# TimoLassmann/tagdust

Hardware: AMD Instinct MI355X
Metric: reads/s (150 bp, 8-barcode arch) (higher is better)
Workload: dtype f32

## Files before the change

### tagdust_amd/csrc/td_jit.h

```cpp
#pragma once
#include <string>
#include <vector>
#include "../../include/tagdust_hip.h"
#include "td_device.h"

struct TdSpecKnobs {
	int block = 512;
	int min_waves = 4;
	int lsum_oob = 1;
	int rt_min = 16;
	int groupcols = 18;
	int groupcols_fwd = 12;
	int prune = 1;
	int prune_sfx = 1;
	int restart = -1;
	int firstseg = -1;
	int trie_sh = 2;
	int profile = 0;
	int prune_stats = -1;
	std::string extra_opts;
};
TdSpecKnobs td_spec_knobs(void);

#define TD_PRUNE_TABLES 16
#define TD_PRUNE_RESTART_MAX 4

struct TdSpecPlan {
	TdSpecKnobs k;
	int S = 0, H = 0, C = 0;
	std::vector<int> col_off, hmm_off;
	std::vector<int> group, group_f;
	std::vector<int> pure_last, drop_m;
	std::vector<int> bw_off;
	int64_t halves = 0;
	std::vector<int> rt, rt_b;
	std::vector<int> base;
	std::vector<float> hi, lo, nv;
	bool trie_on = false;
	int trie_sh = 1, trie_n_share = 0;
	std::vector<int> trie_ord;
	int first_n = 0;
	int prune_segs = 0;
	int sfx_first = 0;
	float prune_z = 0.0f;
	int restart = 0;
};
TdSpecPlan td_spec_plan(const td_model_desc* m, const TdSpecKnobs& k);

float td_spec_prune_z(const td_model_desc* m, int n_seg, int sfx_first);
void td_spec_prune_tables(const td_model_desc* m, const TdSpecPlan& p, int lcap, int stride, std::vector<float>& tab);
void td_spec_layout(TdSpecLayout& L, const TdSpecPlan& p, int lmax);
int td_spec_compile(const td_model_desc* m, const TdSpecPlan& p, int lsum_oob, int window, std::vector<char>& code, std::string& log,
                    uint64_t* key_out = nullptr, bool key_only = false);
int td_spec_compiles_started(void);
```

### tagdust_amd/csrc/td_jit.hip

```cpp
#include <hip/hip_runtime.h>
#include <hip/hiprtc.h>
#include <math.h>
#include <stdio.h>
#include <string.h>
#include <stdlib.h>

#include <atomic>
#include <map>
#include <mutex>
#include <string>
#include <vector>

#include "../../include/tagdust_hip.h"
#include "td_device.h"
#include <unistd.h>
#include <sys/stat.h>
#include <sys/types.h>
#include "td_embedded_src.h"
#include "td_jit.h"

static std::string flit(float v)
{
	if (isinf(v)) return v < 0 ? "(-__builtin_inff())" : "__builtin_inff()";
	if (v != v) return "__builtin_nanf(\"\")";
	char buf[64];
	snprintf(buf, sizeof buf, "%af", (double)v);
	return buf;
}

TdSpecKnobs td_spec_knobs(void)
{
	TdSpecKnobs k;
	auto num = [](const char* name, int unset) { const char* e = getenv(name); return e ? atoi(e) : unset; };
	auto flag = [](const char* name, int unset) -> int { const char* e = getenv(name); return e ? atoi(e) != 0 : unset; };
	if (const int v = num("TD_SPEC_BLOCK", 0); v >= 64 && v <= 1024 && v % 64 == 0) k.block = v;
	if (const int v = num("TD_SPEC_MINWAVES", 0); v >= 1 && v <= 8) k.min_waves = v;
	if (const int v = num("TD_SPEC_GROUPCOLS", 0); v > 0) k.groupcols = v;
	k.groupcols_fwd = num("TD_SPEC_GROUPCOLS_FWD", k.groupcols_fwd);
	k.rt_min = num("TD_SPEC_RT_MIN", k.rt_min);
	k.trie_sh = num("TD_SPEC_TRIE_SH", k.trie_sh);
	k.profile = num("TD_SPEC_PROFILE", k.profile);
	k.lsum_oob = flag("TD_SPEC_LSUM_OOB", k.lsum_oob);
	k.prune = flag("TD_SPEC_PRUNE", k.prune);
	k.prune_sfx = flag("TD_SPEC_PRUNE_SFX", k.prune_sfx);
	k.restart = flag("TD_SPEC_RESTART", k.restart);
	k.firstseg = flag("TD_SPEC_FIRSTSEG", k.firstseg);
	k.prune_stats = flag("TD_SPEC_PRUNE_STATS", k.prune_stats);
	if (const char* e = getenv("TD_SPEC_EXTRA_OPTS")) k.extra_opts = e;
	return k;
}

namespace {
int pure_last(const td_model_desc* m, int j, int col_off)
{
	for (int f = 0; f < m->n_hmm[j]; f++) {
		const int q = col_off + f * m->n_col[j] + m->n_col[j] - 1;
		if (!(m->trans[q * 9 + 4] == -INFINITY) || !(m->trans[q * 9 + 3] == -INFINITY)) return 0;
	}
	return 1;
}

int rt_prefix(const td_model_desc* m, int j, int col_off, int* base , float* hi, float* lo, float* nv, int min_hmms)
{
	const int n = m->n_hmm[j], nc = m->n_col[j];
	if (n < min_hmms) return 0;
	auto match_type = [&](int q, int* b, float* h, float* l, float* v) -> bool {
		const float* e = m->eM + (size_t)q * 5;
		for (int x = 0; x < 4; x++) {
			const float other = e[(x + 1) & 3];
			bool ok = !(e[x] == other);
			for (int y = 0; y < 4 && ok; y++) if (y != x && !(e[y] == other)) ok = false;
			if (ok) { *b = x; *h = e[x]; *l = other; *v = e[4]; return true; }
		}
		return false;
	};
	int b0; float h0, l0, v0;
	if (!match_type(col_off, &b0, &h0, &l0, &v0)) return 0;
	int f = 0;
	for (; f < n; f++) {
		bool ok = true;
		for (int g = 0; g < nc && ok; g++) {
			const int q = col_off + f * nc + g, q0 = col_off + g;
			if (memcmp(m->trans + (size_t)q * 9, m->trans + (size_t)q0 * 9, 36) || memcmp(m->eI + (size_t)q * 5, m->eI + (size_t)q0 * 5, 20) ||
			    memcmp(&m->sM[q], &m->sM[q0], 4) || memcmp(&m->sI[q], &m->sI[q0], 4)) { ok = false; break; }
			int b; float h, l, v;
			if (!match_type(q, &b, &h, &l, &v) || memcmp(&h, &h0, 4) || memcmp(&l, &l0, 4) || memcmp(&v, &v0, 4)) { ok = false; break; }
			base[q] = b;
		}
		if (!ok) break;
	}
	*hi = h0; *lo = l0; *nv = v0;
	return f >= min_hmms ? f : 0;
}

int group_size(int n_hmm, int n_col, int target)
{
	int maxf = target / n_col;
	if (maxf < 1) maxf = 1;
	if (maxf > n_hmm) maxf = n_hmm;
	const int groups = (n_hmm + maxf - 1) / maxf;
	return (n_hmm + groups - 1) / groups;
}

int first_labels(const td_model_desc* m, int firstseg)
{
	const int H = m->H, n0 = m->n_hmm[0];
	const int mode = firstseg >= 0 ? firstseg : H > 32;
	if (!mode) return 0;
	if (n0 < 2 || n0 >= H) return 0;
	for (int v = 0; v < n0; v++)
		for (int u = 0; u < v; u++) if (m->A[u * H + v] == 1.0f) return 0;
	for (int w = n0; w < H; w++) {
		int c = 0;
		for (int u = 0; u < n0; u++) c += m->A[u * H + w] == 1.0f;
		if (c != 0 && c != n0) return 0;
	}
	return n0;
}

bool read_like(const td_model_desc* m, int j, int co)
{
	if (m->n_hmm[j] != 1 || m->n_col[j] != 1) return false;
	const float* t = m->trans + (size_t)co * 9;
	for (int k = 0; k < 9; k++) if (k != TD_II && k != TD_ISKIP && t[k] > -INFINITY) return false;
	return m->sM[co] == -INFINITY && m->sI[co] > -INFINITY && t[TD_II] > -INFINITY && t[TD_ISKIP] > -INFINITY;
}
}

TdSpecPlan td_spec_plan(const td_model_desc* m, const TdSpecKnobs& k)
{
	TdSpecPlan p;
	const int S = m->S, H = m->H, C = m->C;
	p.k = k; p.S = S; p.H = H; p.C = C;
	p.col_off.resize(S); p.hmm_off.resize(S);
	for (int j = 0, co = 0, ho = 0; j < S; co += m->n_hmm[j] * m->n_col[j], ho += m->n_hmm[j], j++) { p.col_off[j] = co; p.hmm_off[j] = ho; }
	p.group.resize(S); p.group_f.resize(S); p.pure_last.resize(S); p.drop_m.resize(S); p.bw_off.resize(H);
	for (int j = 0; j < S; j++) {
		p.group[j] = group_size(m->n_hmm[j], m->n_col[j], k.groupcols);
		p.group_f[j] = group_size(m->n_hmm[j], m->n_col[j], k.groupcols_fwd > 0 ? k.groupcols_fwd : k.groupcols);
		p.pure_last[j] = pure_last(m, j, p.col_off[j]);
	}
	int cols = 0;
	for (int j = 0; j < S; j++) {
		p.drop_m[j] = m->n_col[j] >= 2 && p.pure_last[j];
		for (int f = 0; f < m->n_hmm[j]; f++) { p.bw_off[p.hmm_off[j] + f] = cols; cols += 2 * (m->n_col[j] - p.pure_last[j]) - p.drop_m[j]; }
	}
	p.halves = cols;
	p.rt.assign(S, 0); p.rt_b.assign(S, 0); p.base.assign(C, 0);
	p.hi.assign(S, 0.0f); p.lo.assign(S, 0.0f); p.nv.assign(S, 0.0f);
	for (int j = 0; j < S; j++) {
		const int pre = rt_prefix(m, j, p.col_off[j], p.base.data(), &p.hi[j], &p.lo[j], &p.nv[j], k.rt_min);
		if (pre > 0) {
			p.group_f[j] = p.group[j];
			p.rt[j] = pre / p.group[j] * p.group[j];
			p.rt_b[j] = p.rt[j];
		} else {
			p.rt_b[j] = rt_prefix(m, j, p.col_off[j], p.base.data(), &p.hi[j], &p.lo[j], &p.nv[j], 2);
		}
	}
	{
		const int sh = k.trie_sh;
		bool on = p.rt[0] > 0 && sh >= 1 && m->n_col[0] >= sh + 2;
		std::vector<int> ord;
		int n_share = 0;
		if (on) {
			const int G = p.group[0], NC0 = m->n_col[0];
			std::map<std::vector<int>, std::vector<int>> cls;
			for (int f = 0; f < p.rt[0]; f++) {
				std::vector<int> key;
				for (int g = NC0 - sh; g < NC0; g++) key.push_back(p.base[(size_t)(p.col_off[0] + f * NC0 + g)]);
				cls[key].push_back(f);
			}
			std::vector<int> left;
			for (auto& kv : cls) {
				const std::vector<int>& v = kv.second;
				const size_t full = v.size() / (size_t)G * (size_t)G;
				for (size_t i = 0; i < full; i++) ord.push_back(v[i]);
				for (size_t i = full; i < v.size(); i++) left.push_back(v[i]);
			}
			n_share = (int)ord.size() / G;
			for (int f : left) ord.push_back(f);
			if (n_share == 0) on = false;
		}
		if (!on) { ord.assign(1, 0); n_share = 0; }
		p.trie_on = on; p.trie_sh = on ? sh : 1; p.trie_n_share = n_share; p.trie_ord = ord;
	}
	p.first_n = first_labels(m, k.firstseg);
	p.prune_segs = 0; p.sfx_first = S;
	if (k.prune && H - p.first_n <= 32) {
		int first = -1, last = -1;
		for (int j = 0; j < S; j++) if (read_like(m, j, p.col_off[j])) { if (first < 0) first = j; last = j; }
		if (first > 0) p.prune_segs = first;
		bool single = k.prune_sfx && last >= 0 && last < S - 1;
		for (int j = last + 1; single && j < S; j++) if (m->n_hmm[j] != 1) single = false;
		if (single) p.sfx_first = last + 1;
	}
	p.prune_z = td_spec_prune_z(m, p.prune_segs, p.sfx_first);
	if (p.prune_segs <= 0 || p.prune_segs > TD_PRUNE_RESTART_MAX || (p.sfx_first < S && S - p.sfx_first > TD_PRUNE_RESTART_MAX)) p.restart = 0;
	else if (k.restart >= 0) p.restart = k.restart;
	else p.restart = p.col_off[p.prune_segs] >= 48;
	return p;
}

static std::string td_spec_model_section(const td_model_desc* m, const TdSpecPlan& p, int lsum_oob, int window)
{
	std::string s;
	char buf[256];
	const int S = m->S, H = m->H, C = m->C;
	int req = 0;
	for (int j = 0; j < S; j++) if (m->seg_type[j] == 'F') req += m->finger_len[j];
	snprintf(buf, sizeof buf, "#define TDS_BLOCK %d\n#define TDS_MIN_WAVES %d\n", p.k.block, p.k.min_waves);
	s += buf;
	snprintf(buf, sizeof buf, "#define TDS_LSUM_OOB %d\n", lsum_oob != 0);
	s += buf;
	snprintf(buf, sizeof buf, "#define TDS_WINDOW %d\n", window != 0);
	s += buf;
	snprintf(buf, sizeof buf, "#define TDS_PROFILE %d\n", p.k.profile);
	s += buf;
	snprintf(buf, sizeof buf, "#define TD_S %d\n#define TD_H %d\n#define TD_C %d\n#define TD_REQ_FINGER %d\n", S, H, C, req);
	s += buf;
	s += "struct GCol { float t[9]; float sM, sI; float eM[5]; float eI[5]; };\n";
	auto int_array = [&](const char* name, const std::vector<int>& v) {
		s += std::string("static constexpr int ") + name + "[" + std::to_string(v.size()) + "] = {";
		for (size_t i = 0; i < v.size(); i++) { s += std::to_string(v[i]); if (i + 1 < v.size()) s += ","; }
		s += "};\n";
	};
	int_array("kNHmm", std::vector<int>(m->n_hmm, m->n_hmm + S)); int_array("kNCol", std::vector<int>(m->n_col, m->n_col + S));
	int_array("kColOff", p.col_off); int_array("kHmmOff", p.hmm_off);
	int_array("kRtB", p.rt_b);
	s += std::string("static constexpr bool kTrieOn = ") + (p.trie_on ? "true" : "false") + ";\n";
	s += "static constexpr int kTrieSH = " + std::to_string(p.trie_sh) + ";\n";
	s += "static constexpr int kTrieNShare = " + std::to_string(p.trie_n_share) + ";\n";
	int_array("kTrieOrd", p.trie_ord);
	int_array("kGroup", p.group); int_array("kGroupF", p.group_f); int_array("kPureLast", p.pure_last); int_array("kDropM", p.drop_m); int_array("kBwOff", p.bw_off);
	int_array("kRt", p.rt); int_array("kBase", p.base);
	auto float_array = [&](const char* name, const std::vector<float>& v) {
		s += std::string("static constexpr float ") + name + "[" + std::to_string(v.size()) + "] = {";
		for (size_t i = 0; i < v.size(); i++) { s += flit(v[i]); if (i + 1 < v.size()) s += ","; }
		s += "};\n";
	};
	float_array("kHi", p.hi); float_array("kLo", p.lo); float_array("kNv", p.nv);
	s += "static constexpr float kSkip[" + std::to_string(S) + "] = {";
	for (int j = 0; j < S; j++) { s += flit(m->skip[j]); if (j + 1 < S) s += ","; }
	s += "};\n";
	s += "static constexpr float kBg[5] = {";
	for (int i = 0; i < 5; i++) { s += flit(m->bg[i]); if (i < 4) s += ","; }
	s += "};\n";
	const float stay_arg = (float)(1.0 - (1.0 / (double)(float)m->avg_len));
	const float exit_arg = (float)(1.0 / (double)(float)m->avg_len);
	s += "static constexpr float kRStay = " + flit(stay_arg == 0.0f ? -INFINITY : (float)log((double)stay_arg)) + ";\n";
	s += "static constexpr float kRExit = " + flit(exit_arg == 0.0f ? -INFINITY : (float)log((double)exit_arg)) + ";\n";
	s += "static constexpr GCol kCols[" + std::to_string(C) + "] = {\n";
	for (int k = 0; k < C; k++) {
		s += " {{";
		for (int t = 0; t < 9; t++) { s += flit(m->trans[k * 9 + t]); if (t < 8) s += ","; }
		s += "}," + flit(m->sM[k]) + "," + flit(m->sI[k]) + ",{";
		for (int e = 0; e < 5; e++) { s += flit(m->eM[k * 5 + e]); if (e < 4) s += ","; }
		s += "},{";
		for (int e = 0; e < 5; e++) { s += flit(m->eI[k * 5 + e]); if (e < 4) s += ","; }
		s += "}},\n";
	}
	s += "};\n";
	s += "static constexpr unsigned kHinfo[" + std::to_string(H) + "] = {";
	for (int h = 0; h < H; h++) {
		const int seg = m->label[h] & 0xFFFF, f = (m->label[h] >> 16) & 0x7FFF;
		unsigned v = (unsigned)(unsigned char)m->seg_type[seg] | ((unsigned)seg << 8) | ((unsigned)f << 16);
		if (m->seg_type[seg] == 'B' && f == m->n_hmm[seg] - 1) v |= 0x80000000u;
		snprintf(buf, sizeof buf, "0x%08xu%s", v, h + 1 < H ? "," : "");
		s += buf;
	}
	s += "};\n";
	std::vector<int> poff(H + 1, 0), pidx;
	for (int v = 0; v < H; v++) {
		poff[v] = (int)pidx.size();
		for (int u = 0; u < v; u++) if (m->A[u * H + v] == 1.0f) pidx.push_back(u);
	}
	poff[H] = (int)pidx.size();
	if (pidx.empty()) pidx.push_back(0);
	int_array("kPredOff", poff); int_array("kPredIdx", pidx);
	const int first_n = p.first_n;
	std::vector<int> pfirst(H, 0), poff2(H + 1, 0), pidx2;
	for (int v = 0; v < H; v++) {
		poff2[v] = (int)pidx2.size();
		for (int i = poff[v]; i < poff[v + 1]; i++) {
			if (pidx[i] < first_n) pfirst[v] = 1; else pidx2.push_back(pidx[i]);
		}
	}
	poff2[H] = (int)pidx2.size();
	if (pidx2.empty()) pidx2.push_back(0);
	s += "static constexpr int kFirstN = " + std::to_string(first_n) + ";\n";
	int_array("kPredFirst", pfirst); int_array("kPredOff2", poff2); int_array("kPredIdx2", pidx2);
	std::vector<int> runs;
	for (int v = first_n; v < H; v++) {
		bool same = v > first_n && pfirst[v] == pfirst[v - 1] && poff2[v + 1] - poff2[v] == poff2[v] - poff2[v - 1];
		for (int k = 0; same && k < poff2[v + 1] - poff2[v]; k++) same = pidx2[poff2[v] + k] == pidx2[poff2[v - 1] + k];
		if (!same) runs.push_back(v - first_n);
	}
	runs.push_back(H - first_n);
	s += "static constexpr int kPruneSegs = " + std::to_string(p.prune_segs) + ";\n";
	s += "static constexpr int kSfxFirst = " + std::to_string(p.sfx_first) + ";\n";
	s += "static constexpr float kPruneZ = " + flit(p.prune_z) + ";\n";
	if (p.k.prune_stats >= 0) s += std::string("#define TDS_PRUNE_STATS ") + (p.k.prune_stats ? "1" : "0") + "\n";
	s += std::string("#ifndef TDS_RESTART\n#define TDS_RESTART ") + (p.restart ? "1" : "0") + "\n#endif\n";
	s += "static constexpr int kNRuns = " + std::to_string((int)runs.size() - 1) + ";\n";
	int_array("kRunOff", runs);
	return s;
}

static std::string td_spec_full_source(const td_model_desc* m, const TdSpecPlan& p, int lsum_oob, int window)
{
	std::string src = "#ifndef __HIPCC_RTC__\n#include <hip/hip_runtime.h>\n#endif\n#include <stdint.h>\n";
	src += kSrcDeviceH;
	src += "\n";
	src += kSrcArtifact;
	src += "\n";
	src += td_spec_model_section(m, p, lsum_oob, window);
	src += kSrcSpecKernel;
	return src;
// ... 193 lines not shown
```

### tagdust_amd/csrc/td_spec_kernel.inc

```

#ifndef TDS_BLOCK
#define TDS_BLOCK 512
#endif
#ifndef TDS_MIN_WAVES
#define TDS_MIN_WAVES 4
#endif
#define TDS_REG_H 32
#define TDS_WPB (TDS_BLOCK / TD_WAVE)
#define NEG_INF (-__builtin_inff())
#define DEV __device__ __forceinline__

#define MODE_GET_LABEL 1
#define MODE_ARCH_COMP 5
#define OUT_SUCCESS 0
#define OUT_ARCH_MISMATCH 1
#define OUT_TOO_SHORT 2
#define OUT_BAR_FINGER_NOT_FOUND 3
#define OUT_MATCHES_ARTIFACTS 5
#define OUT_LOW_COMPLEXITY 6
#define N_OUTCOME_SLOTS 8
#define TDS_DIAG(k) (N_OUTCOME_SLOTS + 256 + ((k) - 192))

#ifndef TDS_LSUM_OOB
#define TDS_LSUM_OOB 1
// ... 109 lines not shown
	const int c1 = (e0 == e1) + (e2 == e1) + (e3 == e1);
	const int c2 = (e0 == e2) + (e1 == e2) + (e3 == e2);
	const int c3 = (e0 == e3) + (e1 == e3) + (e2 == e3);
	float lo = e0;
	int best = c0;
	if (c1 > best) { lo = e1; best = c1; }
	if (c2 > best) { lo = e2; best = c2; }
	if (c3 > best) { lo = e3; best = c3; }
	float r = lo;
	if (e0 != lo) r = k.m0 ? e0 : r;
	if (e1 != lo) r = k.m1 ? e1 : r;
	if (e2 != lo) r = k.m2 ? e2 : r;
	if (e3 != lo) r = k.m3 ? e3 : r;
	if (e4 != lo) r = k.m4 ? e4 : r;
	return r;
}
#define EMIT_M(col, k) emit(kCols[col].eM[0], kCols[col].eM[1], kCols[col].eM[2], kCols[col].eM[3], kCols[col].eM[4], k)
#define EMIT_I(col, k) emit(kCols[col].eI[0], kCols[col].eI[1], kCols[col].eI[2], kCols[col].eI[3], kCols[col].eI[4], k)
DEV float emit_rt(const int b, const float hi, const float lo, const float nv, const BaseMask& k, const int x)
{
	const float r = (x == b) ? hi : lo;
	return k.m4 ? nv : r;
}

#ifndef TDS_PROFILE
#define TDS_PROFILE 0
#endif
#define TDS_PHASE(k) do { if (TDS_PROFILE) { const long long t_ = (long long)__builtin_readcyclecounter(); \
	if (lane == 0) atomicAdd(&ka.counters[TDS_DIAG(240 + (k))], (unsigned long long)(t_ - tprof)); tprof = t_; } } while (0)

#ifndef TDS_WINDOW
#define TDS_WINDOW 0
#endif
constexpr bool kMaskDP = TD_H - kFirstN <= TDS_REG_H;

struct Wv {
	uint32_t* pmask;
	int nwm;
	uint8_t* slot;
	int lane, len, lmax, tmax, tmin;
	float* bm;
	uint8_t* ba;
	int cut;
	int cutS;
	const float* wa;
	const float* wb;
	int sstop;
	int sstopS;
	const float* wc;
	const float* wd;
	mutable int bad;
	bool rb_on, rf_on;
	float* rs;
	float* hb;
	int rWf;
	int rW;
	const float* bwt;
	const float* fbs;
	unsigned long long* stats;
	long long* tprof;
	const float* ptab;
	int pstride;
	const float* qr;
	const float* pr;
};

#ifndef TDS_LATE_CS
#define TDS_LATE_CS 1
#endif
#ifndef TDS_PF_DIST
#define TDS_PF_DIST 4
#endif
#ifndef TDS_PF_COLS
#define TDS_PF_COLS 2
#endif
#ifndef TDS_LDP
#define TDS_LDP 2
#endif
#ifndef TDS_LDT
#define TDS_LDT 4
#endif
#ifndef TDS_SCAN_B
#define TDS_SCAN_B 8
#endif
#ifndef TDS_PRUNE_TT
#define TDS_PRUNE_TT (-88.0f)
#endif
#ifndef TDS_PRUNE_MARGIN
#define TDS_PRUNE_MARGIN 1
#endif
#ifndef TDS_PRUNE_BGAP
#define TDS_PRUNE_BGAP 5.0f
#endif
#ifndef TDS_PRUNE_STATS
#define TDS_PRUNE_STATS 0
#endif

constexpr int cmin(int a, int b) { return a < b ? a : b; }
constexpr int pf_dist(int cols, bool rt) { return (!rt && cols <= TDS_PF_COLS) ? TDS_PF_DIST : 1; }
template <int D> struct IC { static constexpr int v = D; };
constexpr bool label_leading(int h)
{
	for (int j = 0; j < kPruneSegs; j++) if (h >= kHmmOff[j] && h < kHmmOff[j] + kNHmm[j]) return true;
	return false;
}
template <int PD, int D, typename F>
DEV void ring_block(F& step, const int base)
{
	if constexpr (D < PD) { step(IC<D>{}, base + D); ring_block<PD, D + 1>(step, base); }
}
template <int PD, int D, typename F>
DEV void ring_rest(F& step, const int base, const int iend)
{
	if constexpr (D < PD - 1) { if (base + D <= iend) { step(IC<D>{}, base + D); ring_rest<PD, D + 1>(step, base, iend); } }
}

template <int J, bool RT>
DEV void bwd_row(const int fa, const float (&Mn)[kNCol[J]], const float (&In)[kNCol[J]], const float Pn,
                 const BaseMask& kc, const int c, const BaseMask& kx, const int xi, SV (&Mc)[kNCol[J]], SV (&Ic)[kNCol[J]])
{
#define EM(gcol, mask, xval) (RT ? emit_rt(kBase[colr + (gcol)], kHi[J], kLo[J], kNv[J], mask, xval) : EMIT_M(col0 + (gcol), mask))
	constexpr int NC = kNCol[J];
	constexpr int K = NC - 1;
	const int col0 = kColOff[J] + (RT ? 0 : fa) * NC;
	const int colr = kColOff[J] + fa * NC;
	(void)colr;
	SV Dp = sv_none();
	{
		const int q = col0 + K;
		const SV M = addc(sv(Pn), kCols[q].t[7]);
		SV I = addc(sv(Pn), kCols[q].t[8]);
		I = lsum(I, addv(addc(sv(Mn[K]), kCols[q].t[4]), EM(K, kc, c)));
		I = lsum(I, addv(addc(sv(In[K]), kCols[q].t[3]), EMIT_I(q, kc)));
		Mc[K] = M; Ic[K] = I;
	}
#pragma unroll
	for (int g = K - 1; g >= 0; --g) {
		const int q = col0 + g;
		const float epc = EM(g + 1, kc, c);
		const float eic = EMIT_I(q, kc);
		SV M = addc(addv(sv(Mn[g + 1]), epc), kCols[q].t[0]);
		SV I = addv(addc(sv(In[g]), kCols[q].t[3]), eic);
		lsum2(M, addc(sv(Pn), kCols[q].t[7]), I, addc(sv(Pn), kCols[q].t[8]));
		lsum2(M, addc(addv(sv(In[g]), eic), kCols[q].t[1]), I, addv(addc(sv(Mn[g + 1]), kCols[q].t[4]), epc));
		SV D = addc(Dp, kCols[q].t[5]);
		lsum2(M, addc(Dp, kCols[q].t[2]), D, addc(addv(Mc[g + 1], EM(g + 1, kx, xi)), kCols[q].t[6]));
		Mc[g] = M; Ic[g] = I; Dp = D;
	}
#undef EM
}

template <int J, bool RT, int GT, int GB>
DEV void bwd_cols(const int fa, const float (&Mn)[kNCol[J]], const float (&In)[kNCol[J]], const float Pn,
                  const BaseMask& kc, const int c, const BaseMask& kx, const int xi, SV (&Mc)[kNCol[J]], SV (&Ic)[kNCol[J]], SV& Dp)
{
#define EM(gcol, mask, xval) (RT ? emit_rt(kBase[colr + (gcol)], kHi[J], kLo[J], kNv[J], mask, xval) : EMIT_M(col0 + (gcol), mask))
	constexpr int NC = kNCol[J];
	constexpr int K = NC - 1;
	const int col0 = kColOff[J] + (RT ? 0 : fa) * NC;
	const int colr = kColOff[J] + fa * NC;
	(void)colr;
	if constexpr (GT == K) {
		const int q = col0 + K;
		const SV M = addc(sv(Pn), kCols[q].t[7]);
		SV I = addc(sv(Pn), kCols[q].t[8]);
		I = lsum(I, addv(addc(sv(Mn[K]), kCols[q].t[4]), EM(K, kc, c)));
// ... 559 lines not shown
			ub_term(mi, ni, addc(Io, kCols[q].t[3]));
			ub_term(mi, ni, addc(Mo, kCols[q].t[1]));
			ub_term(md, nd, addc(Mcu, kCols[qp].t[2]));
			ub_term(md, nd, addc(Du, kCols[qp].t[5]));
			Mc[g] = nm ? si(NEG_INF, ub_done(mm, nm) + em) : si_none();
			Ic[g] = ni ? si(NEG_INF, ub_done(mi, ni) + ei) : si_none();
			Dc = nd ? si(NEG_INF, ub_done(md, nd)) : si_none();
		}
	}
#pragma unroll
	for (int g = 0; g < NC; g++) {
		Mlo[g] = Mc[g].z ? NEG_INF : Mc[g].lo; Mhi[g] = Mc[g].z ? NEG_INF : Mc[g].hi;
		Ilo[g] = Ic[g].z ? NEG_INF : Ic[g].lo; Ihi[g] = Ic[g].z ? NEG_INF : Ic[g].hi;
	}
}

template <int J, int GC>
DEV void fstair_dispatch(const int gc, float (&Mlo)[kNCol[J]], float (&Mhi)[kNCol[J]], float (&Ilo)[kNCol[J]], float (&Ihi)[kNCol[J]], const float Pm, const BaseMask& kc)
{
	if constexpr (kNCol[J] > TDS_STAIR_STATIC_COLS) {
		fstair_step<J, -2>(gc, Mlo, Mhi, Ilo, Ihi, Pm, kc);
	} else if constexpr (GC <= kNCol[J]) {
		if (gc == GC) fstair_step<J, GC>(gc, Mlo, Mhi, Ilo, Ihi, Pm, kc);
		else fstair_dispatch<J, GC + 1>(gc, Mlo, Mhi, Ilo, Ihi, Pm, kc);
	}
}

template <int J>
DEV void fwd_stair(const Wv& w, const uint8_t* __restrict__ codes, const float* __restrict__ P, const int q_lo, const int q_hi)
{
	constexpr int NC = kNCol[J];
	float hi0 = NEG_INF;
	{
		const float* gf = w.ptab + (int64_t)(12 + J - kSfxFirst) * w.pstride;
		const int t = q_lo - 1;
		for (int k0 = 1; k0 <= t; k0 += 8) {
			float pr[8];
#pragma unroll
			for (int u = 0; u < 8; u++) { const int k = k0 + u; pr[u] = w.pr[((k <= t) ? t - k : 0) * TD_WAVE + w.lane]; }
			__builtin_amdgcn_sched_barrier(0);
#pragma unroll
			for (int u = 0; u < 8; u++) { const int k = k0 + u; if (k <= t) hi0 = fmaxf(hi0, uload(gf, k) + pr[u]); }
		}
		hi0 = fminf(hi0 + (__logf((float)(t > 1 ? t : 1)) + 0.02f), w.fbs[t]);
	}
	float Mlo[NC], Mhi[NC], Ilo[NC], Ihi[NC];
#pragma unroll
	for (int g = 0; g < NC; g++) { Mlo[g] = NEG_INF; Ilo[g] = NEG_INF; Mhi[g] = hi0; Ihi[g] = hi0; }
	int gc = 0;
	int closed_at = -1;
	auto close_check = [&](const int steps_done) __attribute__((always_inline)) {
		if (gc < NC) {
			bool cl = true;
#pragma unroll
			for (int g = 0; g < NC; g++) if (g == gc) cl = same(si(Mlo[g], Mhi[g])) && same(si(Ilo[g], Ihi[g]));
			if (__builtin_amdgcn_ballot_w64(!cl) == 0) { gc++; if (gc == NC) closed_at = steps_done; }
		}
	};
	int c_n = codes[q_lo * TD_WAVE + w.lane];
	float Pm_n = P[(q_lo - 1) * TD_WAVE + w.lane];
	for (int i = q_lo; i < q_hi; ++i) {
		const int c = c_n;
		const float Pm = Pm_n;
		{
			const int ip = (i + 1 < q_hi) ? i + 1 : i;
			c_n = codes[ip * TD_WAVE + w.lane];
			Pm_n = P[(ip - 1) * TD_WAVE + w.lane];
		}
		close_check(i - q_lo); close_check(i - q_lo);
		fstair_dispatch<J, 0>(gc, Mlo, Mhi, Ilo, Ihi, Pm, mk_mask(c));
	}
	close_check(q_hi - q_lo); close_check(q_hi - q_lo);
	if (gc < NC) w.bad |= 32;
	if (TDS_PRUNE_STATS && w.lane == 0) {
		const int st = closed_at >= 0 ? closed_at : q_hi - q_lo;
		atomicAdd(&w.stats[TDS_DIAG(194)], (unsigned long long)st); atomicAdd(&w.stats[TDS_DIAG(195)], 1ull);
		atomicMax(&w.stats[TDS_DIAG(192)], (unsigned long long)st);
	}
	float* rs = w.rs + (int64_t)kColOff[J] * 2 * TD_WAVE + w.lane;
#pragma unroll
	for (int g = 0; g < NC; g++) { rs[(2 * g) * TD_WAVE] = Mlo[g]; rs[(2 * g + 1) * TD_WAVE] = Ilo[g]; }
}

template <int J, int NF, bool RT>
DEV void fwd_group(const Wv& w, const uint8_t* __restrict__ codes, const float* __restrict__ P,
                   float* __restrict__ Cs, const float* __restrict__ PB, const uint8_t* __restrict__ BW,
                   float* __restrict__ DP, float* __restrict__ TOTAL, const float b, const int f0)
{
	const bool first = (f0 == 0);
#define EM(gcol, mask, xval) (RT ? emit_rt(kBase[colr + (gcol)], kHi[J], kLo[J], kNv[J], mask, xval) : EMIT_M(col0 + (gcol), mask))
	constexpr int NC = kNCol[J];
	constexpr int K = NC - 1;
	constexpr bool pure = kPureLast[J] != 0;
	constexpr int NS = NC - kPureLast[J];
	constexpr int DM = kDropM[J];
	constexpr int NSF = NS - DM;
	constexpr int ROWH = 2 * NS - DM;
	constexpr int NQ = NSF / 2;
	constexpr int NT = NSF & 1;
	constexpr bool skip_live = LIVE(kSkip[J]);
	float Mp[NF][NC], Ip[NF][NC], tot[NF];
#pragma unroll
	for (int f = 0; f < NF; f++) {
		tot[f] = NEG_INF;
#pragma unroll
		for (int g = 0; g < NC; g++) { Mp[f][g] = NEG_INF; Ip[f][g] = NEG_INF; }
	}
	if (TDS_RESTART && J >= kSfxFirst && w.rf_on) {
		const float* rs = w.rs + (int64_t)kColOff[J] * 2 * TD_WAVE + w.lane;
#pragma unroll
		for (int g = 0; g < NC; g++) { Mp[0][g] = rs[(2 * g) * TD_WAVE]; Ip[0][g] = rs[(2 * g + 1) * TD_WAVE]; }
	}
	constexpr bool p_init = (J == 0);
	const bool resumed = TDS_RESTART && (J >= kSfxFirst) && w.rf_on;
	const int i0 = resumed ? w.sstop - (TD_S - 1 - J) * (w.rWf + 1) : 1;
	float Pm = p_init ? 0.0f : P[(i0 - 1) * TD_WAVE + w.lane];
	constexpr int PD = pf_dist(NF * NC, RT);
	const int pmax = (w.tmax >= 1) ? w.tmax : 1;
	int c_q[PD];
	float Pi_q[PD], cs_q[PD], pb_q[PD], bm_q[PD], ik_q[PD][NF];
	int ba_q[PD];
	float MB_q[PD][NF][NSF + 1], IB_q[PD][NF][NSF + 1];
	constexpr bool pb_init = (J == TD_S - 1);
#define PBR(pos) (pb_init ? (((pos) == w.len + 1) ? 0.0f : NEG_INF) : PB[(pos) * TD_WAVE + w.lane])
#define BWROW(f_, pos_) (BW + ((int64_t)kBwOff[kHmmOff[J] + f0 + (f_)] * w.lmax + (int64_t)((pos_) - 1) * ROWH) * (TD_WAVE * 4))
#define TDS_FWD_FILL(d, p_raw) { \
		const int p_ = ((p_raw) <= pmax) ? (p_raw) : pmax; \
		c_q[d] = codes[p_ * TD_WAVE + w.lane]; \
		Pi_q[d] = p_init ? NEG_INF : P[p_ * TD_WAVE + w.lane]; \
		if (!first) cs_q[d] = Cs[p_ * TD_WAVE + w.lane]; \
		if (pure) pb_q[d] = PBR(p_ + 1); \
		if (own_sum && !first) { bm_q[d] = w.bm[p_ * TD_WAVE + w.lane]; ba_q[d] = w.ba[p_ * TD_WAVE + w.lane]; } \
		const bool rows_ = !((J >= kSfxFirst) && p_ < w.sstop);    \
_Pragma("unroll") \
		for (int f = 0; f < NF; f++) { \
			if (DM && rows_) ik_q[d][f] = ld1(BWROW(f, p_) + NSF * (TD_WAVE * 8), w.lane); \
			if (PD > 1 && rows_) { \
_Pragma("unroll") \
				for (int q = 0; q < NQ; q++) { \
					MB_q[d][f][2 * q] = ldk(BWROW(f, p_) + q * (TD_WAVE * 16), w.lane, 16, 0); IB_q[d][f][2 * q] = ldk(BWROW(f, p_) + q * (TD_WAVE * 16), w.lane, 16, 1); \
					MB_q[d][f][2 * q + 1] = ldk(BWROW(f, p_) + q * (TD_WAVE * 16), w.lane, 16, 2); IB_q[d][f][2 * q + 1] = ldk(BWROW(f, p_) + q * (TD_WAVE * 16), w.lane, 16, 3); \
				} \
				if (NT) { MB_q[d][f][NSF - 1] = ldk(BWROW(f, p_) + NQ * (TD_WAVE * 16), w.lane, 8, 0); IB_q[d][f][NSF - 1] = ldk(BWROW(f, p_) + NQ * (TD_WAVE * 16), w.lane, 8, 1); } \
			} \
		} \
	}
	constexpr bool own_sum = (J == 0) && (kFirstN > 0);
	float lacc[NF];
	uint32_t mbits[NF];
#pragma unroll
	for (int f = 0; f < NF; f++) { lacc[f] = 0.0f; mbits[f] = 0u; }
#pragma unroll
	for (int d = 0; d < PD; d++) {
		cs_q[d] = NEG_INF; pb_q[d] = 0.0f; bm_q[d] = -1.0f; ba_q[d] = 0;
#pragma unroll
		for (int f = 0; f < NF; f++) ik_q[d][f] = NEG_INF;
		TDS_FWD_FILL(d, i0 + d)
	}

	const int iend = (J < kPruneSegs && w.cut < w.tmax) ? w.cut : w.tmax;
	const int itail = (J == kPruneSegs && kPruneSegs > 0) ? w.cut + 1 : w.tmax + 1;
	(void)itail;
	if (i0 > 1 && kMaskDP && !own_sum) {
#pragma unroll
		for (int f = 0; f < NF; f++) {
			if (w.lane == 0) for (int wd = 0; wd < ((i0 - 1) >> 5); wd++) w.pmask[(kHmmOff[J] + f0 + f) * w.nwm + wd] = 0u;
			mbits[f] = 0u;
		}
	}
	auto step_cs = [&](auto dtag, auto cstag, const int i) __attribute__((always_inline)) {
		constexpr int d_ = decltype(dtag)::v;
		constexpr bool want_cs = decltype(cstag)::v != 0;
		const int c = c_q[d_];
		const float Pi = Pi_q[d_];
		const float pb = pb_q[d_];
		SV cs; cs.v = cs_q[d_]; cs.z = RT ? false : first;
		float bm = bm_q[d_];
		int ba = ba_q[d_];
		f32x4 cb[NF][NQ + 1];
		f32x2 ct[NF];
		const bool sfx_skip = (J >= kSfxFirst) && i < w.sstop;
		float ik[NF];
#pragma unroll
		for (int f = 0; f < NF; f++) {
			if constexpr (PD == 1) {
				const uint8_t* bw = BW + ((int64_t)kBwOff[kHmmOff[J] + f0 + f] * w.lmax + (int64_t)(i - 1) * ROWH) * (TD_WAVE * 4);
				if (!sfx_skip) {
#pragma unroll
					for (int p = 0; p < NQ; p++) cb[f][p] = ld4(bw + p * (TD_WAVE * 16), w.lane);
					if (NT) ct[f] = ld2(bw + NQ * (TD_WAVE * 16), w.lane);
				}
			} else {
#pragma unroll
				for (int p = 0; p < NQ; p++) cb[f][p] = f32x4{ MB_q[d_][f][2 * p], IB_q[d_][f][2 * p], MB_q[d_][f][2 * p + 1], IB_q[d_][f][2 * p + 1] };
				if (NT) ct[f] = f32x2{ MB_q[d_][f][NSF - 1], IB_q[d_][f][NSF - 1] };
			}
			ik[f] = ik_q[d_][f];
		}
		TDS_FWD_FILL(d_, i + PD)
		const int dn_ = (d_ + 1) % PD;
		const int c_n = c_q[dn_];
		const float pb_n = pb_q[dn_];
		float ik_n[NF];
#pragma unroll
		for (int f = 0; f < NF; f++) ik_n[f] = ik_q[dn_][f];
		float lpost[NF];
#pragma unroll
		for (int f = 0; f < NF; f++) lpost[f] = NEG_INF;
		const bool tail = (J == kPruneSegs && kPruneSegs > 0) && i >= itail;
		if (i <= w.len) {
			const SV PmS = sv(tail ? NEG_INF : Pm);
			const SV PiS = sv(tail ? NEG_INF : Pi);
			const BaseMask kc = mk_mask(c);
#pragma unroll
			for (int f = 0; f < NF; f++) {
				const int col0 = kColOff[J] + (RT ? 0 : (f0 + f)) * NC;
				const int colr = kColOff[J] + (f0 + f) * NC;
				(void)colr;
				const int h = kHmmOff[J] + f0 + f;
				SV Mc[NC], Ic[NC];
				SV Dc = sv_none();
				const float ei0 = EMIT_I(col0, kc);
				{
					const int q = col0;
					const SV M = addv(addc(PmS, kCols[q].sM), EM(0, kc, c));
					SV I = addc(PmS, kCols[q].sI);
					if (tail && LIVE(kCols[q].sI)) {
						if (!(Ip[f][0] + kCols[q].t[3] >= uload(w.wa, i))) w.bad |= 1;
					}
					I = lsum(I, addc(sv(Ip[f][0]), kCols[q].t[3]));
					I = lsum(I, addc(sv(Mp[f][0]), kCols[q].t[1]));
					I = addv(I, ei0);
					if (want_cs) { cs = lsum(cs, addc(M, kCols[q].t[7])); cs = lsum(cs, addc(I, kCols[q].t[8])); }
					Mc[0] = M; Ic[0] = I;
				}
#pragma unroll
				for (int g = 1; g <= K; ++g) {
					const int q = col0 + g, qp = q - 1;
					SV M = addc(PmS, kCols[q].sM);
					SV I = addc(PmS, kCols[q].sI);
					lsum2(M, addc(sv(Mp[f][g - 1]), kCols[qp].t[0]), I, addc(sv(Ip[f][g]), kCols[q].t[3]));
					lsum2(M, addc(sv(Ip[f][g - 1]), kCols[qp].t[4]), I, addc(sv(Mp[f][g]), kCols[q].t[1]));
					SV D = addc(Mc[g - 1], kCols[qp].t[2]);
					lsum2(M, addc(Dc, kCols[qp].t[6]), D, addc(Dc, kCols[qp].t[5]));
					M = addv(M, EM(g, kc, c));
					I = addv(I, EMIT_I(q, kc));
					if (want_cs) { cs = lsum(cs, addc(M, kCols[q].t[7])); cs = lsum(cs, addc(I, kCols[q].t[8])); }
					Mc[g] = M; Ic[g] = I; Dc = D;
				}
				if (tail && skip_live) { if (!(cs.v >= uload(w.wb, i))) w.bad |= 2; }
				if (want_cs) cs = lsum(cs, addc(PiS, kSkip[J]));
				if (!sfx_skip) {
				float MB[NC], IB[NC];
#pragma unroll
				for (int p = 0; p < NQ; p++) {
					const f32x4 v = cb[f][p];
					MB[2 * p] = v.x; IB[2 * p] = v.y; MB[2 * p + 1] = v.z; IB[2 * p + 1] = v.w;
				}
				if (NT) { MB[NSF - 1] = ct[f].x; IB[NSF - 1] = ct[f].y; }
				if constexpr (DM != 0) {
					constexpr int g = K - 1;
					const int q = col0 + g;
					const bool nxt = i < w.len;
					const int cx = (i < w.tmax) ? c_n : 0;
					const BaseMask kn = mk_mask(cx);
					SV MnK = addc(sv(pb_n), kCols[col0 + K].t[7]);
					if (!MnK.z) MnK.v = nxt ? MnK.v : NEG_INF;
					const float InK = nxt ? ik_n[f] : NEG_INF;
					SV Mr = addc(addv(MnK, EM(K, kn, cx)), kCols[q].t[0]);
					Mr = lsum(Mr, addc(sv(pb), kCols[q].t[7]));
					Mr = lsum(Mr, addc(addv(sv(InK), EMIT_I(q, kn)), kCols[q].t[1]));
					MB[g] = Mr.v; IB[g] = ik[f];
				}
				if (pure) {
					MB[K] = pb + kCols[col0 + K].t[7];
					IB[K] = pb + kCols[col0 + K].t[8];
				}
				constexpr bool want_tt = kNHmm[J] > 1;
				SV acc = sv_none(), tt = sv(tot[f]);
#pragma unroll
				for (int g = 0; g <= K; ++g) {
					const SV pm = subv(addv(Mc[g], MB[g]), b);
					if (want_tt && g == 0) tt = lsum(tt, pm);
					acc = lsum(acc, pm);
					if (want_tt && g == 0) tt = lsum(tt, subv(addv(addv(addc(PmS, kCols[col0].sI), ei0), IB[0]), b));
					acc = lsum(acc, subv(addv(Ic[g], IB[g]), b));
				}
				if (want_tt) tot[f] = tt.v;
				if (own_sum) {
					lacc[f] = post_prob(acc.v) + lacc[f];
					if (lacc[f] > bm) { bm = lacc[f]; ba = h; }
				} else if (kMaskDP) {
					lpost[f] = acc.v;
				} else {
					DP[((int64_t)(i - 1) * TD_H + h) * TD_WAVE + w.lane] = post_prob(acc.v);
				}
				}
#pragma unroll
				for (int g = 0; g < NC; g++) { Mp[f][g] = Mc[g].v; Ip[f][g] = Ic[g].v; }
			}
			if (want_cs) Cs[i * TD_WAVE + w.lane] = cs.v;
			if (own_sum) { w.bm[i * TD_WAVE + w.lane] = bm; w.ba[i * TD_WAVE + w.lane] = (uint8_t)ba; }
		}
		if (kMaskDP && !own_sum) {
#pragma unroll
			for (int f = 0; f < NF; f++) {
				const bool on = lpost[f] > -103.98f;
				const bool any_on = __builtin_amdgcn_ballot_w64(on) != 0;
				if (any_on) {
					float pp = 0.0f;
					if (on) pp = (float)exp((double)lpost[f]);
					if (i <= w.len) DP[((int64_t)(i - 1) * TD_H + kHmmOff[J] + f0 + f) * TD_WAVE + w.lane] = pp;
				}
				mbits[f] |= (any_on ? 1u : 0u) << ((i - 1) & 31);
				if ((((i - 1) & 31) == 31) || i == iend) {
					if (w.lane == 0) w.pmask[(kHmmOff[J] + f0 + f) * w.nwm + ((i - 1) >> 5)] = mbits[f];
					mbits[f] = 0u;
				}
			}
		}
		Pm = Pi;
	};
	{
		constexpr bool cs_late = TDS_LATE_CS && (J == TD_S - 1) && !((J == kPruneSegs && kPruneSegs > 0) && skip_live);
		auto step = [&](auto dtag, const int i) __attribute__((always_inline)) { step_cs(dtag, IC<1>{}, i); };
		auto step_nocs = [&](auto dtag, const int i) __attribute__((always_inline)) { step_cs(dtag, IC<0>{}, i); };
		int base = i0;
		if constexpr (cs_late) {
			const int i_cs = (w.tmin < iend) ? w.tmin : iend;
			for (; base + PD - 1 < i_cs; base += PD) ring_block<PD, 0>(step_nocs, base);
		}
		for (; base + PD - 1 <= iend; base += PD) ring_block<PD, 0>(step, base);
		ring_rest<PD, 0>(step, base, iend);
	}
	if (J < kPruneSegs && iend < w.tmax) {
		if (kMaskDP && !own_sum && w.lane == 0) {
#pragma unroll
			for (int f = 0; f < NF; f++)
				for (int wd = ((iend - 1) >> 5) + 1; wd < w.nwm; wd++) w.pmask[(kHmmOff[J] + f0 + f) * w.nwm + wd] = 0u;
		}
		if (kNHmm[J] > 1 && w.len > iend) {
#pragma unroll
			for (int f = 0; f < NF; f++) if (!(tot[f] >= TDS_PRUNE_TT)) w.bad |= 4;
		}
	}
	if (kNHmm[J] > 1) {
#pragma unroll
		for (int f = 0; f < NF; f++) TOTAL[(kHmmOff[J] + f0 + f) * TD_WAVE + w.lane] = tot[f];
	}
#undef EM
#undef PBR
#undef BWROW
#undef TDS_FWD_FILL
}

template <int J, int F0>
DEV void fwd_groups(const Wv& w, const uint8_t* __restrict__ codes, const float* __restrict__ P,
                    float* __restrict__ Cs, const float* __restrict__ PB, const uint8_t* __restrict__ BW,
                    float* __restrict__ DP, float* __restrict__ TOTAL, const float b)
{
	if constexpr (TDS_RESTART && F0 == 0 && J >= kSfxFirst) {
		if (w.rf_on) {
			const int q_hi = w.sstop - (TD_S - 1 - J) * (w.rWf + 1);
			fwd_stair<J>(w, codes, P, q_hi - w.rWf, q_hi);
		}
	}
	if constexpr (F0 == 0 && kRt[J] > 0) {
		for (int f0 = 0; f0 < kRt[J]; f0 += kGroupF[J]) fwd_group<J, kGroupF[J], true>(w, codes, P, Cs, PB, BW, DP, TOTAL, b, f0);
		fwd_groups<J, kRt[J]>(w, codes, P, Cs, PB, BW, DP, TOTAL, b);
	} else if constexpr (F0 < kNHmm[J]) {
		constexpr int NF = cmin(kGroupF[J], kNHmm[J] - F0);
		fwd_group<J, NF, false>(w, codes, P, Cs, PB, BW, DP, TOTAL, b, F0);
		fwd_groups<J, F0 + NF>(w, codes, P, Cs, PB, BW, DP, TOTAL, b);
	}
}

template <int J>
DEV void fwd_segments(const Wv& w, const uint8_t* __restrict__ codes, float* __restrict__ SF, const float* __restrict__ SB,
                      int rowlen, const uint8_t* __restrict__ BW, float* __restrict__ DP, float* __restrict__ TOTAL, const float b)
{
	if constexpr (J < TD_S) {
		fwd_groups<J, 0>(w, codes, SF + (int64_t)J * rowlen, SF + (int64_t)(J + 1) * rowlen, SB + (int64_t)(J + 1) * rowlen,
		                 BW, DP, TOTAL, b);
		if (TDS_PROFILE == 2 && J < 8) { const long long t_ = (long long)__builtin_readcyclecounter(); if (w.lane == 0) atomicAdd(&w.stats[TDS_DIAG(216 + J)], (unsigned long long)(t_ - *w.tprof)); *w.tprof = t_; }
		fwd_segments<J + 1>(w, codes, SF, SB, rowlen, BW, DP, TOTAL, b);
	}
}

constexpr bool path_word_trivial(int k)
{
	for (int b = 0; b < 4; b++) {
		const int v = kFirstN + 4 * k + b;
		if (v < TD_H && (kPredFirst[v] != 0 || kPredOff2[v + 1] != kPredOff2[v])) return false;
	}
	return true;
}
constexpr uint32_t path_word_identity(int k)
{
	uint32_t w = 0;
	for (int b = 0; b < 4; b++) w |= (uint32_t)((kFirstN + 4 * k + b) & 0xFF) << (8 * b);
	return w;
}

DEV int prune_scan(const float thr, const int len, const int tmax, const float* __restrict__ fbt, const float* __restrict__ bwt)
{
	int cl = 1;
	for (int i0 = 2; i0 <= tmax; i0 += TDS_SCAN_B) {
		float g[TDS_SCAN_B];
#pragma unroll
		for (int k = 0; k < TDS_SCAN_B; k++) {
			const int i = i0 + k;
			const int mm = (i <= len) ? len - i : 0;
			g[k] = bwt[mm];
		}
		__builtin_amdgcn_sched_barrier(0);
#pragma unroll
		for (int k = 0; k < TDS_SCAN_B; k++) g[k] = uload(fbt, i0 + k) + g[k];
#pragma unroll
		for (int k = 0; k < TDS_SCAN_B; k++) {
			const int i = i0 + k;
			if (i <= len && i <= tmax && g[k] > thr) cl = i;
		}
	}
#pragma unroll
	for (int o = 32; o >= 1; o >>= 1) cl = max(cl, __shfl_xor(cl, o));
	return __builtin_amdgcn_readfirstlane(cl);
}

DEV float leading_bwd_bound(const Wv& w, const int i)
{
	float hb = NEG_INF;
	for (int k0 = 0; i + 1 + k0 <= w.tmax + 1; k0 += TDS_SCAN_B) {
		float q[TDS_SCAN_B];
#pragma unroll
		for (int u = 0; u < TDS_SCAN_B; u++) {
			const int pos = i + 1 + k0 + u;
			q[u] = w.qr[(pos <= w.tmax + 1 ? pos : w.tmax + 1) * TD_WAVE + w.lane];
		}
		__builtin_amdgcn_sched_barrier(0);
#pragma unroll
		for (int u = 0; u < TDS_SCAN_B; u++) {
			const int k = k0 + u, pos = i + 1 + k;
			float g = uload(w.ptab + (int64_t)8 * w.pstride, k);
#pragma unroll
			for (int J = 1; J < 4; J++) if (J < kPruneSegs) g = fmaxf(g, uload(w.ptab + (int64_t)(8 + J) * w.pstride, k));
			if (pos <= w.len + 1) hb = fmaxf(hb, g + q[u]);
		}
	}
	return hb + (__logf((float)(w.len - i + 1)) + 0.02f);
}
DEV int refine_cut(const Wv& w, int cq, const float thr, const float* __restrict__ fbt, const float* __restrict__ bwt)
{
	while (cq > 1) {
		bool viol = false;
		if (cq <= w.len) {
// ... 885 lines not shown
```

Baseline: 84.41 million.

## Share identical prefix columns across HMMs in forward groups

At plan time, finds for each HMM how many leading columns have transitions and emissions identical to the previous HMM in the same segment. The forward kernel then maps shared columns to a single computed state slot, so those cells are not recomputed, and re-packs group sizes by a column budget that counts only the unshared columns. The aim is to remove redundant forward DP arithmetic and register pressure for barcode HMMs with common prefixes. It adds constexpr slot-mapping complexity and can change group sizes, which affects unrolling and register use.

Result: slower. 82.69 million (-2.0%).

```diff
diff --git a/tagdust_amd/csrc/td_jit.h b/tagdust_amd/csrc/td_jit.h
--- a/tagdust_amd/csrc/td_jit.h
+++ b/tagdust_amd/csrc/td_jit.h
@@ -16,6 +16,7 @@
 	int restart = -1;
 	int firstseg = -1;
 	int trie_sh = 2;
+	int fwd_share = 1;
 	int profile = 0;
 	int prune_stats = -1;
 	std::string extra_opts;
@@ -30,6 +31,8 @@
 	int S = 0, H = 0, C = 0;
 	std::vector<int> col_off, hmm_off;
 	std::vector<int> group, group_f;
+	std::vector<int> fwd_share;
+	std::vector<int> group_fn;
 	std::vector<int> pure_last, drop_m;
 	std::vector<int> bw_off;
 	int64_t halves = 0;
diff --git a/tagdust_amd/csrc/td_jit.hip b/tagdust_amd/csrc/td_jit.hip
--- a/tagdust_amd/csrc/td_jit.hip
+++ b/tagdust_amd/csrc/td_jit.hip
@@ -39,6 +39,7 @@
 	k.groupcols_fwd = num("TD_SPEC_GROUPCOLS_FWD", k.groupcols_fwd);
 	k.rt_min = num("TD_SPEC_RT_MIN", k.rt_min);
 	k.trie_sh = num("TD_SPEC_TRIE_SH", k.trie_sh);
+	k.fwd_share = flag("TD_SPEC_FWD_SHARE", k.fwd_share);
 	k.profile = num("TD_SPEC_PROFILE", k.profile);
 	k.lsum_oob = flag("TD_SPEC_LSUM_OOB", k.lsum_oob);
 	k.prune = flag("TD_SPEC_PRUNE", k.prune);
@@ -156,6 +157,28 @@
 			p.rt_b[j] = p.rt[j];
 		} else {
 			p.rt_b[j] = rt_prefix(m, j, p.col_off[j], p.base.data(), &p.hi[j], &p.lo[j], &p.nv[j], 2);
+		}
+	}
+	p.fwd_share.assign(H, 0); p.group_fn.assign(H, 0);
+	if (k.fwd_share) {
+		for (int j = 0; j < S; j++) {
+			const int n = m->n_hmm[j], nc = m->n_col[j], co = p.col_off[j], ho = p.hmm_off[j];
+			for (int f = 1; f < n; f++) {
+				int s = 0;
+				for (; s < nc - 1; s++) {
+					const size_t q = (size_t)(co + f * nc + s), q0 = q - (size_t)nc;
+					if (memcmp(m->trans + q * 9, m->trans + q0 * 9, 36) || memcmp(m->eM + q * 5, m->eM + q0 * 5, 20) ||
+					    memcmp(m->eI + q * 5, m->eI + q0 * 5, 20) || memcmp(&m->sM[q], &m->sM[q0], 4) || memcmp(&m->sI[q], &m->sI[q0], 4)) break;
+				}
+				p.fwd_share[ho + f] = s;
+			}
+			const int budget = p.rt[j] > 0 ? p.group[j] * nc : (k.groupcols_fwd > 0 ? k.groupcols_fwd : k.groupcols);
+			for (int f = p.rt[j]; f < n;) {
+				int nf = 1, cols = nc;
+				while (f + nf < n && cols + nc - p.fwd_share[ho + f + nf] <= budget) { cols += nc - p.fwd_share[ho + f + nf]; nf++; }
+				p.group_fn[ho + f] = nf;
+				f += nf;
+			}
 		}
 	}
 	{
@@ -234,6 +257,7 @@
 	int_array("kTrieOrd", p.trie_ord);
 	int_array("kGroup", p.group); int_array("kGroupF", p.group_f); int_array("kPureLast", p.pure_last); int_array("kDropM", p.drop_m); int_array("kBwOff", p.bw_off);
 	int_array("kRt", p.rt); int_array("kBase", p.base);
+	if (p.k.fwd_share) { s += "#define TDS_FWD_SHARE 1\n"; int_array("kShareF", p.fwd_share); int_array("kGroupFN", p.group_fn); }
 	auto float_array = [&](const char* name, const std::vector<float>& v) {
 		s += std::string("static constexpr float ") + name + "[" + std::to_string(v.size()) + "] = {";
 		for (size_t i = 0; i < v.size(); i++) { s += flit(v[i]); if (i + 1 < v.size()) s += ","; }
diff --git a/tagdust_amd/csrc/td_spec_kernel.inc b/tagdust_amd/csrc/td_spec_kernel.inc
--- a/tagdust_amd/csrc/td_spec_kernel.inc
+++ b/tagdust_amd/csrc/td_spec_kernel.inc
@@ -215,6 +215,9 @@
 #endif
 #ifndef TDS_SCAN_B
 #define TDS_SCAN_B 8
+#endif
+#ifndef TDS_FWD_SHARE
+#define TDS_FWD_SHARE 0
 #endif
 #ifndef TDS_PRUNE_TT
 #define TDS_PRUNE_TT (-88.0f)
@@ -940,7 +943,24 @@
 	for (int g = 0; g < NC; g++) { rs[(2 * g) * TD_WAVE] = Mlo[g]; rs[(2 * g + 1) * TD_WAVE] = Ilo[g]; }
 }
 
-template <int J, int NF, bool RT>
+template <int NF, int NC> struct FwdSlots { int sh[NF]; int s[NF][NC]; int nd; };
+template <int J, int NF, int F0S>
+constexpr FwdSlots<NF, kNCol[J]> fwd_slots()
+{
+	FwdSlots<NF, kNCol[J]> r{};
+	for (int f = 0; f < NF; f++) {
+#if TDS_FWD_SHARE
+		r.sh[f] = (F0S < 0 || f == 0) ? 0 : kShareF[kHmmOff[J] + F0S + f];
+#else
+		r.sh[f] = 0;
+#endif
+		for (int g = 0; g < kNCol[J]; g++) r.s[f][g] = (g < r.sh[f]) ? r.s[f - 1][g] : r.nd++;
+	}
+	return r;
+}
+template <int J, int NF, int F0S> static constexpr FwdSlots<NF, kNCol[J]> kFwdSlots = fwd_slots<J, NF, F0S>();
+
+template <int J, int NF, bool RT, int F0S = -1>
 DEV void fwd_group(const Wv& w, const uint8_t* __restrict__ codes, const float* __restrict__ P,
                    float* __restrict__ Cs, const float* __restrict__ PB, const uint8_t* __restrict__ BW,
                    float* __restrict__ DP, float* __restrict__ TOTAL, const float b, const int f0)
@@ -957,17 +977,17 @@
 	constexpr int NQ = NSF / 2;
 	constexpr int NT = NSF & 1;
 	constexpr bool skip_live = LIVE(kSkip[J]);
-	float Mp[NF][NC], Ip[NF][NC], tot[NF];
-#pragma unroll
-	for (int f = 0; f < NF; f++) {
-		tot[f] = NEG_INF;
-#pragma unroll
-		for (int g = 0; g < NC; g++) { Mp[f][g] = NEG_INF; Ip[f][g] = NEG_INF; }
-	}
+#define FSL kFwdSlots<J, NF, F0S>
+	constexpr int ND = FSL.nd;
+	float Mp[ND], Ip[ND], tot[NF];
+#pragma unroll
+	for (int f = 0; f < NF; f++) tot[f] = NEG_INF;
+#pragma unroll
+	for (int d = 0; d < ND; d++) { Mp[d] = NEG_INF; Ip[d] = NEG_INF; }
 	if (TDS_RESTART && J >= kSfxFirst && w.rf_on) {
 		const float* rs = w.rs + (int64_t)kColOff[J] * 2 * TD_WAVE + w.lane;
 #pragma unroll
-		for (int g = 0; g < NC; g++) { Mp[0][g] = rs[(2 * g) * TD_WAVE]; Ip[0][g] = rs[(2 * g + 1) * TD_WAVE]; }
+		for (int g = 0; g < NC; g++) { Mp[g] = rs[(2 * g) * TD_WAVE]; Ip[g] = rs[(2 * g + 1) * TD_WAVE]; }
 	}
 	constexpr bool p_init = (J == 0);
 	const bool resumed = TDS_RESTART && (J >= kSfxFirst) && w.rf_on;
@@ -1070,41 +1090,47 @@
 			const SV PmS = sv(tail ? NEG_INF : Pm);
 			const SV PiS = sv(tail ? NEG_INF : Pi);
 			const BaseMask kc = mk_mask(c);
+			SV Mcd[ND], Icd[ND], Dcd[ND];
 #pragma unroll
 			for (int f = 0; f < NF; f++) {
 				const int col0 = kColOff[J] + (RT ? 0 : (f0 + f)) * NC;
 				const int colr = kColOff[J] + (f0 + f) * NC;
 				(void)colr;
 				const int h = kHmmOff[J] + f0 + f;
-				SV Mc[NC], Ic[NC];
-				SV Dc = sv_none();
+				const int sh = FSL.sh[f];
+				const int* sl = FSL.s[f];
 				const float ei0 = EMIT_I(col0, kc);
 				{
 					const int q = col0;
-					const SV M = addv(addc(PmS, kCols[q].sM), EM(0, kc, c));
-					SV I = addc(PmS, kCols[q].sI);
-					if (tail && LIVE(kCols[q].sI)) {
-						if (!(Ip[f][0] + kCols[q].t[3] >= uload(w.wa, i))) w.bad |= 1;
+					if (0 >= sh) {
+						const SV M = addv(addc(PmS, kCols[q].sM), EM(0, kc, c));
+						SV I = addc(PmS, kCols[q].sI);
+						if (tail && LIVE(kCols[q].sI)) {
+							if (!(Ip[sl[0]] + kCols[q].t[3] >= uload(w.wa, i))) w.bad |= 1;
+						}
+						I = lsum(I, addc(sv(Ip[sl[0]]), kCols[q].t[3]));
+						I = lsum(I, addc(sv(Mp[sl[0]]), kCols[q].t[1]));
+						I = addv(I, ei0);
+						Mcd[sl[0]] = M; Icd[sl[0]] = I; Dcd[sl[0]] = sv_none();
 					}
-					I = lsum(I, addc(sv(Ip[f][0]), kCols[q].t[3]));
-					I = lsum(I, addc(sv(Mp[f][0]), kCols[q].t[1]));
-					I = addv(I, ei0);
-					if (want_cs) { cs = lsum(cs, addc(M, kCols[q].t[7])); cs = lsum(cs, addc(I, kCols[q].t[8])); }
-					Mc[0] = M; Ic[0] = I;
+					if (want_cs) { cs = lsum(cs, addc(Mcd[sl[0]], kCols[q].t[7])); cs = lsum(cs, addc(Icd[sl[0]], kCols[q].t[8])); }
 				}
 #pragma unroll
 				for (int g = 1; g <= K; ++g) {
 					const int q = col0 + g, qp = q - 1;
-					SV M = addc(PmS, kCols[q].sM);
-					SV I = addc(PmS, kCols[q].sI);
-					lsum2(M, addc(sv(Mp[f][g - 1]), kCols[qp].t[0]), I, addc(sv(Ip[f][g]), kCols[q].t[3]));
-					lsum2(M, addc(sv(Ip[f][g - 1]), kCols[qp].t[4]), I, addc(sv(Mp[f][g]), kCols[q].t[1]));
-					SV D = addc(Mc[g - 1], kCols[qp].t[2]);
-					lsum2(M, addc(Dc, kCols[qp].t[6]), D, addc(Dc, kCols[qp].t[5]));
-					M = addv(M, EM(g, kc, c));
-					I = addv(I, EMIT_I(q, kc));
-					if (want_cs) { cs = lsum(cs, addc(M, kCols[q].t[7])); cs = lsum(cs, addc(I, kCols[q].t[8])); }
-					Mc[g] = M; Ic[g] = I; Dc = D;
+					if (g >= sh) {
+						const SV Dc = Dcd[sl[g - 1]];
+						SV M = addc(PmS, kCols[q].sM);
+						SV I = addc(PmS, kCols[q].sI);
+						lsum2(M, addc(sv(Mp[sl[g - 1]]), kCols[qp].t[0]), I, addc(sv(Ip[sl[g]]), kCols[q].t[3]));
+						lsum2(M, addc(sv(Ip[sl[g - 1]]), kCols[qp].t[4]), I, addc(sv(Mp[sl[g]]), kCols[q].t[1]));
+						SV D = addc(Mcd[sl[g - 1]], kCols[qp].t[2]);
+						lsum2(M, addc(Dc, kCols[qp].t[6]), D, addc(Dc, kCols[qp].t[5]));
+						M = addv(M, EM(g, kc, c));
+						I = addv(I, EMIT_I(q, kc));
+						Mcd[sl[g]] = M; Icd[sl[g]] = I; Dcd[sl[g]] = D;
+					}
+					if (want_cs) { cs = lsum(cs, addc(Mcd[sl[g]], kCols[q].t[7])); cs = lsum(cs, addc(Icd[sl[g]], kCols[q].t[8])); }
 				}
 				if (tail && skip_live) { if (!(cs.v >= uload(w.wb, i))) w.bad |= 2; }
 				if (want_cs) cs = lsum(cs, addc(PiS, kSkip[J]));
@@ -1138,11 +1164,11 @@
 				SV acc = sv_none(), tt = sv(tot[f]);
 #pragma unroll
 				for (int g = 0; g <= K; ++g) {
-					const SV pm = subv(addv(Mc[g], MB[g]), b);
+					const SV pm = subv(addv(Mcd[sl[g]], MB[g]), b);
 					if (want_tt && g == 0) tt = lsum(tt, pm);
 					acc = lsum(acc, pm);
 					if (want_tt && g == 0) tt = lsum(tt, subv(addv(addv(addc(PmS, kCols[col0].sI), ei0), IB[0]), b));
-					acc = lsum(acc, subv(addv(Ic[g], IB[g]), b));
+					acc = lsum(acc, subv(addv(Icd[sl[g]], IB[g]), b));
 				}
 				if (want_tt) tot[f] = tt.v;
 				if (own_sum) {
@@ -1154,9 +1180,9 @@
 					DP[((int64_t)(i - 1) * TD_H + h) * TD_WAVE + w.lane] = post_prob(acc.v);
 				}
 				}
-#pragma unroll
-				for (int g = 0; g < NC; g++) { Mp[f][g] = Mc[g].v; Ip[f][g] = Ic[g].v; }
-			}
+			}
+#pragma unroll
+			for (int d = 0; d < ND; d++) { Mp[d] = Mcd[d].v; Ip[d] = Icd[d].v; }
 			if (want_cs) Cs[i * TD_WAVE + w.lane] = cs.v;
 			if (own_sum) { w.bm[i * TD_WAVE + w.lane] = bm; w.ba[i * TD_WAVE + w.lane] = (uint8_t)ba; }
 		}
@@ -1207,6 +1233,7 @@
 		for (int f = 0; f < NF; f++) TOTAL[(kHmmOff[J] + f0 + f) * TD_WAVE + w.lane] = tot[f];
 	}
 #undef EM
+#undef FSL
 #undef PBR
 #undef BWROW
 #undef TDS_FWD_FILL
@@ -1227,8 +1254,13 @@
 		for (int f0 = 0; f0 < kRt[J]; f0 += kGroupF[J]) fwd_group<J, kGroupF[J], true>(w, codes, P, Cs, PB, BW, DP, TOTAL, b, f0);
 		fwd_groups<J, kRt[J]>(w, codes, P, Cs, PB, BW, DP, TOTAL, b);
 	} else if constexpr (F0 < kNHmm[J]) {
+#if TDS_FWD_SHARE
+		constexpr int NF = kGroupFN[kHmmOff[J] + F0];
+		fwd_group<J, NF, false, F0>(w, codes, P, Cs, PB, BW, DP, TOTAL, b, F0);
+#else
 		constexpr int NF = cmin(kGroupF[J], kNHmm[J] - F0);
 		fwd_group<J, NF, false>(w, codes, P, Cs, PB, BW, DP, TOTAL, b, F0);
+#endif
 		fwd_groups<J, F0 + NF>(w, codes, P, Cs, PB, BW, DP, TOTAL, b);
 	}
 }
```
